# siyuanwu99/pred-occ-planner

Hardware: AMD Instinct MI355X
Metric: replans/sec (SOGM update + QP: full replan = SOGM update + A* + corridors + QP + deconfliction), 128-agent batch per GPU, 200x200x200x20 voxel grid; aggregate over all agents (higher is better)
Workload: dtype f32 occupancy / f64 planning; 1 GPU; 128 agents/GPU x 1 GPU, 200x200x200x20 SOGM, sim_fkpcp-style moving cylinders, batched ADMM QP (BASELINE configs[2] per GPU); agents_total=128, cloud_points=622040, cylinders=555, map_input_staleness_ticks=0, parallelism=agents sharded x1, 1 all-gather/tick, exchange=local, sogm_grids_per_agent=3, sogm_reset=sparse (logged 32-byte sectors), sogm_cell_order=2x2x2 tiles, map_update=at the start of the tick

## Files before the change

### pred-occ-planner_amd/csrc/sogm_device.hpp

```cpp
#pragma once

#include <hip/hip_fp16.h>
#include <hip/hip_runtime.h>

#include <cstdlib>

#include <new>
#include <stdint.h>

#include "../../include/sogm_abi_debug.h"
#include "../../include/sogm_detmath.h"
#include "sogm_gridpool.hpp"
#include "sogm_resources.hpp"

namespace sogm {
typedef float vfloat4 __attribute__((ext_vector_type(4)));

struct GridGeom {
  int   L, W, H, T;
  int   V;
  float res;
  float rx, ry, rz;
  float dt;
  float risk_threshold;
// ... 391 lines not shown
  for (int k = 0; k < piece; ++k) t0 += r.duration[k];
  const double tf = t0 + r.duration[piece], dur = tf - t0, s = (tt - t0) / dur;
  const double A[5][5] = {{1, -4, 6, -4, 1}, {0, 4, -12, 12, -4}, {0, 0, 6, -12, 6},
                          {0, 0, 0, 4, -4},  {0, 0, 0, 0, 1}};
  const double S0[5] = {1, s, s * s, s * s * s, (s * s) * (s * s)};
  const double S1[5] = {0, 1, 2 * s, 3 * (s * s), 4 * (s * s * s)};
  const double S2[5] = {0, 0, 2, 6 * s, 12 * (s * s)};
  const double *c    = r.cpts + piece * 15;
  for (int d = 0; d < 3; ++d) {
    double p = 0, v = 0, a = 0;
    for (int j = 0; j < 5; ++j) {
      double b = 0;
      for (int q = 0; q < 5; ++q) b += c[q * 3 + d] * A[q][j];
      p += b * S0[j];
      v += b * S1[j];
      a += b * S2[j];
    }
    out[d]     = p;
    out[3 + d] = v / dur;
    out[6 + d] = a / (dur * dur);
  }
  return true;
}
__device__ inline bool traj_eval_record(const SogmTrajRecord &r, double t_abs, double out[9]) {
  return traj_eval_relative(r, t_abs - r.time_start, out);
}
}

#define SOGM_TUNING_TABLE(X)                                                                                             \
  X(GROUPS, "groups", 2, 1, 64)                     \
  X(SPEC_ASTAR, "spec_astar", 1, 0, 1)             \
  X(CLEAR_GATE_FRAC, "clear_gate_frac", 1, 0, 1)  \
  X(QP_WGS, "qp_wgs", 0, 0, 1024)                     \
  X(FINISH_WGS, "finish_wgs", 0, 0, 64)             \
  X(CORRIDOR_WGS, "corridor_wgs", 0, 0, 65536)      \
  X(QP_ABLATE, "qp_ablate", 0, 0, 255)               \
  X(CLEAR_WGS, "clear_wgs", 0, 0, 65536)               \
  X(CLEAR_THROTTLE, "clear_throttle", 0, 0, 64)     \
  X(CLEAR_NT, "clear_nt", 1, 0, 1)                 \
  X(CLEAR_WIDE_WGS, "clear_wide_wgs", 256, 0, 65536)   \
  X(CLEAR_WIDE_BOUND, "clear_wide_bound", 0, 0, 64)  \
  X(CLEAR_HEAD_GB, "clear_head_gb", 1.0e9, 0, 1.0e12)   \
  X(CLEAR_EARLY, "clear_early", 0, 0, 1)           \
  X(CLEAR_RETIRE_AT_END, "clear_retire_at_end", 0, 0, 1)   \
  X(RESET_WGS, "reset_wgs", 32, 0, 4096)              \
  X(RESET_LANES, "reset_lanes", 0, 0, 4)           \
  X(RESET_UNROLL, "reset_unroll", 0, 0, 8)         \
  X(RESET_LATE, "reset_late", 1, 0, 1)             \
  X(STAMP_WGS, "stamp_wgs", 256, 0, 4096)             \
  X(STAMP_BITS_WGS, "stamp_bits_wgs", 0, 0, 4096)     \
  X(STAMP_LDS_LOG, "stamp_lds_log", 1, 0, 1)          \
  X(STAMP_CACHED, "stamp_cached", 0, 0, 1)            \
  X(STAMP_LDS_KB, "stamp_lds_kb", 0, 0, 64)                \
  X(SPLAT_WGS, "splat_wgs", 256, 0, 65536)             \
  X(SPLAT_OVERLAP, "splat_overlap", 1, 0, 1)       \
  X(PRESTAMP_BITS, "prestamp_bits", 32, 0, 1024)      \
  X(PRESTAMP_MARKS, "prestamp_marks", 64, 0, 1024)    \
  X(PRESTAMP_WGS, "prestamp_wgs", 0, 0, 65536)         \
  X(PRESTAMP_GATE_FRAC, "prestamp_gate_frac", 0.9, 0, 1)  \
  X(PRESTAMP_STREAM, "prestamp_stream", 1, 0, 1)  \
  X(PRESTAMP_LATE_AGENTS, "prestamp_late_agents", 8, 0, 65536)    \
  X(PRESTAMP_LATE_BITS, "prestamp_late_bits", 128, 0, 4096)      \
  X(PRESTAMP_LATE_MARKS, "prestamp_late_marks", 256, 0, 4096)    \
  X(FLIGHT_QP_UNITS, "flight_qp_units", 4, 1, 13)            \
  X(FLIGHT_SEARCH_UNITS, "flight_search_units", 2, 1, 13)    \
  X(FLIGHT_MAP_UNITS, "flight_map_units", 4, 1, 13)          \
  X(FLIGHT_MASKS, "flight_masks", 1, 0, 1)                   \
  X(FLIGHT_SPEC, "flight_spec", 1, 0, 1)                     \
  X(FLIGHT_RESET, "flight_reset", 8, 1, 256)                 \
  X(FLIGHT_BITS, "flight_bits", 16, 1, 256)                  \
  X(FLIGHT_MARKS, "flight_marks", 32, 1, 256)                \
  X(FLIGHT_SPLAT, "flight_splat", 4, 1, 64)                  \
  X(FLIGHT_ADMIT, "flight_admit", 48, 1, 65536)              \
  X(FLIGHT_PACE_US, "flight_pace_us", 20, 0, 100000)         \
  X(FLIGHT_HEADS, "flight_heads", 32, 1, 4096)               \
  X(FLIGHT_URGENT, "flight_urgent", 8, 0, 65536)            \
  X(FLIGHT_URGENT_WAVES, "flight_urgent_waves", 4096, 1, 4096)  \
  X(FLIGHT_URGENT_FINE, "flight_urgent_fine", 4, 1, 16)      \
  X(FLIGHT_GATE_PACE_US, "flight_gate_pace_us", 20, 0, 100000)   \
  X(FLIGHT_NEIGHBOUR_LAG, "flight_neighbour_lag", 2, 1, 2)  \
  X(FLIGHT_ENGINES, "flight_engines", 4, 1, 4)              \
  X(FLIGHT_ENGINE_FIRST, "flight_engine_first", 0, 0, 3)    \
  X(FLIGHT_EXCHANGE_UNITS, "flight_exchange_units", 0, 0, 4)  \
  X(FLIGHT_LIGHT_PER_CU, "flight_light_per_cu", 4, 1, 4)    \
  X(FLIGHT_MAP_PER_CU, "flight_map_per_cu", 8, 1, 8)        \
  X(UPDATE_FLOW, "update_flow", 0, 0, 1)                    \
  X(UPDATE_BITS, "update_bits", 16, 1, 256)                  \
  X(UPDATE_MARKS, "update_marks", 64, 1, 256)                \
  X(UPDATE_SPLAT, "update_splat", 40, 1, 64)                 \
  X(UPDATE_WGS, "update_wgs", 0, 0, 65536)                   \
  X(UPDATE_CHUNK, "update_chunk", 1, 1, 64)                  \
  X(UPDATE_CACHED, "update_cached", 0, 0, 1)                 \
  X(UPDATE_ORDER, "update_order", 1, 0, 1)
enum {
#define X(id, name, dflt, lo, hi) SOGM_TUNE_##id,
  SOGM_TUNING_TABLE(X)
#undef X
  SOGM_TUNE_N
};

struct sogm_ctx {
  sogm::Resources res;
  SogmSpec       spec;
  sogm::GridGeom geom;
  int            n_agents;
  int            device;
// ... 177 lines not shown
```

### pred-occ-planner_amd/csrc/sogm_map.hip

```cpp
#include <hip/hip_runtime.h>

#include <utility>
#include <vector>

#include "sogm_device.hpp"
#include "sogm_fsm.hpp"
#include "sogm_planner.hpp"

namespace sogm {

#define SOGM_MAX_CYL_LDS 1024

__device__ inline void cross3f(const float a[3], const float b[3], float o[3]) {
  o[0] = a[1] * b[2] - a[2] * b[1];
  o[1] = a[2] * b[0] - a[0] * b[2];
  o[2] = a[0] * b[1] - a[1] * b[0];
}
__device__ inline void quat_rotate_f(float qw, const float qv[3], const float v[3], float o[3]) {
  float uv[3], w2[3];
  cross3f(qv, v, uv);
  for (int k = 0; k < 3; ++k) uv[k] += uv[k];
  cross3f(qv, uv, w2);
  for (int k = 0; k < 3; ++k) o[k] = (v[k] + qw * uv[k]) + w2[k];
}
// ... 244 lines not shown
  if (f.cb.bounds) {
    stamp_bits_blocks<WAVE_DEDUPE>(g, f.cloud, f.cb, agent, sub, n_sub, pose[0], pose[1], pose[2], mask, lane);
  } else {
    const int begin = f.cloud_range[agent * 2], end = f.cloud_range[agent * 2 + 1];
    stamp_bits_range(g, f.cloud, begin + sub * 64 + lane, end, n_sub * 64, pose[0], pose[1], pose[2], mask);
  }
}
__global__ __launch_bounds__(64) void k_stamp_bits(GridGeom g, const float *__restrict__ cloud,
                                                   const int32_t *__restrict__ cloud_range,
                                                   const float *__restrict__ poses, unsigned *__restrict__ bits,
                                                   int words_per_agent, int agent0) {
  const MapFrame  f{.cloud = cloud, .cloud_range = cloud_range, .cb = {}};
  const MapTarget t{.bits = bits, .words = words_per_agent, .poses = const_cast<float *>(poses)};
  bits_ticket(g, f, t, (int)blockIdx.y + agent0, (int)blockIdx.x, (int)gridDim.x, (int)threadIdx.x);
}

__global__ __launch_bounds__(64) void k_stamp_bits_blocks(GridGeom g, const float *__restrict__ cloud, CloudBlocks cb,
                                                          const float *__restrict__ poses, unsigned *__restrict__ bits,
                                                          int words_per_agent) {
  const MapFrame  f{.cloud = cloud, .cb = cb};
  const MapTarget t{.bits = bits, .words = words_per_agent, .poses = const_cast<float *>(poses)};
  bits_ticket<true>(g, f, t, (int)blockIdx.y, (int)blockIdx.x, (int)gridDim.x, (int)threadIdx.x);
}
__global__ __launch_bounds__(64) void k_block_bounds(const float *__restrict__ cloud, int n_points, int block_points,
                                                     float *__restrict__ out) {
  const int b = blockIdx.x, lane = threadIdx.x;
  const int beg = b * block_points, end = beg + block_points < n_points ? beg + block_points : n_points;
  float xlo = INFINITY, xhi = -INFINITY, ylo = INFINITY, yhi = -INFINITY;
  for (int j = beg + lane; j < end; j += 64) {
    const float x = cloud[(size_t)j * 3], y = cloud[(size_t)j * 3 + 1];
    xlo = fminf(xlo, x);
    xhi = fmaxf(xhi, x);
    ylo = fminf(ylo, y);
    yhi = fmaxf(yhi, y);
  }
#pragma unroll
  for (int d = 32; d >= 1; d >>= 1) {
    xlo = fminf(xlo, __shfl_xor(xlo, d, 64));
    xhi = fmaxf(xhi, __shfl_xor(xhi, d, 64));
    ylo = fminf(ylo, __shfl_xor(ylo, d, 64));
    yhi = fmaxf(yhi, __shfl_xor(yhi, d, 64));
  }
  if (lane == 0) reinterpret_cast<float4 *>(out)[b] = make_float4(xlo, xhi, ylo, yhi);
}

#ifdef SOGM_PROFILE_PRESTAMP
__device__ unsigned long long g_ps_prof[12];
#define PS_CLK() wall_clock64()
#define PS_ADD(i, v) do { if (threadIdx.x == 0) atomicAdd(&g_ps_prof[i], (unsigned long long)(v)); } while (0)
#else
#define PS_CLK() 0ll
#define PS_ADD(i, v) do { } while (0)
#endif
template <bool CACHED>
__device__ __forceinline__ void stamp_marks_trips(const GridGeom &g, void *__restrict__ grid,
                                                  unsigned *__restrict__ bits, int words_per_agent,
                                                  const SogmCylinder *__restrict__ cyl, int n_cyl,
                                                  const float *__restrict__ poses,
                                                  const CylCand *__restrict__ cand_all,
                                                  const int *__restrict__ n_cand, int agent, const MarkLog &lg,
                                                  int w_first, int w_stride, CylCand *cand_lds = nullptr,
                                                  int cand_lds_cap = 0, unsigned *lds_secs = nullptr) {
  const int      kept   = n_cand[agent];
  const bool     culled = kept <= SOGM_MAX_CYL_LDS;
  const int      n_lds  = culled ? kept : 0;
  const int      n_loop = culled ? kept : n_cyl;
  const CylCand *cand   = cand_all + (size_t)agent * SOGM_MAX_CYL_LDS;
  const float   *pose   = poses + agent * 3;
  const float    p0 = pose[0], p1 = pose[1], p2 = pose[2];
  char          *base = reinterpret_cast<char *>(grid) + (size_t)agent * g.T * (size_t)g.V * (g.half ? 2 : 4);
  unsigned      *mask = bits + (size_t)agent * words_per_agent;
  const int      lane = threadIdx.x;
  unsigned n_marks = 0, n_logged = 0;
  int n_staged = 0;
  bool staged  = cand_lds == nullptr;
  for (int w0 = w_first; w0 < words_per_agent; w0 += w_stride) {
    uint4 *wp = reinterpret_cast<uint4 *>(mask + w0) + lane;
    uint4  w4 = *wp;
    if ((w4.x | w4.y | w4.z | w4.w) != 0u) *wp = make_uint4(0u, 0u, 0u, 0u);
    const int c0 = __popc(w4.x), c1 = c0 + __popc(w4.y), c2 = c1 + __popc(w4.z), cnt = c2 + __popc(w4.w);
    int       inc = cnt;
#pragma unroll
    for (int d = 1; d < 64; d <<= 1) {
      const int o = __shfl_up(inc, d, 64);
      if (lane >= d) inc += o;
    }
    const int excl  = inc - cnt;
    const int total = __shfl(inc, 63, 64);
    if (total > 0 && !staged) {
      n_staged            = n_lds < cand_lds_cap ? n_lds : cand_lds_cap;
      const uint4 *src    = reinterpret_cast<const uint4 *>(cand);
      uint4       *dst    = reinterpret_cast<uint4 *>(cand_lds);
      const int    pieces = n_staged * (int)(sizeof(CylCand) / 16);
      for (int q = lane; q < pieces; q += 64) dst[q] = src[q];
      __syncthreads();
      staged = true;
    }
    for (int b0 = 0; b0 < total; b0 += 64) {
      const int  i      = b0 + lane;
      const bool active = i < total;
      int lo = 0, hi = 63;
#pragma unroll
      for (int it = 0; it < 6; ++it) {
        const int mid = (lo + hi + 1) >> 1;
        const int em  = __shfl(excl, mid, 64);
        if (em <= i) lo = mid; else hi = mid - 1;
      }
      const int      own = lo;
      const int      r   = i - __shfl(excl, own, 64);
      const unsigned q0 = (unsigned)__shfl((int)w4.x, own, 64), q1 = (unsigned)__shfl((int)w4.y, own, 64);
      const unsigned q2 = (unsigned)__shfl((int)w4.z, own, 64), q3 = (unsigned)__shfl((int)w4.w, own, 64);
      const int      k0 = __shfl(c0, own, 64), k1 = __shfl(c1, own, 64), k2 = __shfl(c2, own, 64);
      const int esh = g.half ? 4 : 3;
      int       v   = 0;
      if (active) {
        const int sel = r < k0 ? 0 : r < k1 ? 1 : r < k2 ? 2 : 3;
        unsigned  wv  = sel == 0 ? q0 : sel == 1 ? q1 : sel == 2 ? q2 : q3;
        int       rr  = r - (sel == 0 ? 0 : sel == 1 ? k0 : sel == 2 ? k1 : k2);
        while (rr-- > 0) wv &= wv - 1;
        v = (w0 + own * 4 + sel) * 32 + __builtin_ctz(wv);
      }
      if (active) {
        cell_st(base, (size_t)v, 1.0F, g.half);
        ++n_marks;
      }
      float cx, cy, cz;
      g.corner_of(g.logical_of(v), pose, cx, cy, cz);
      float vx = 0.f, vy = 0.f;
      bool found = !active;
      [[maybe_unused]] const long long ps_w0 = PS_CLK();
      auto walk_filtered = [&](const auto *cl) __attribute__((always_inline)) {
        float xlo = active ? cx : INFINITY, xhi = active ? cx : -INFINITY;
        float ylo = active ? cy : INFINITY, yhi = active ? cy : -INFINITY;
#pragma unroll
        for (int d = 32; d >= 1; d >>= 1) {
          xlo = fminf(xlo, __shfl_xor(xlo, d, 64));
          xhi = fmaxf(xhi, __shfl_xor(xhi, d, 64));
          ylo = fminf(ylo, __shfl_xor(ylo, d, 64));
          yhi = fmaxf(yhi, __shfl_xor(yhi, d, 64));
        }
        bool done = false;
        for (int c0 = 0; c0 < n_loop && !done; c0 += 64) {
          bool maybe = false;
          if (c0 + lane < n_loop) {
            const CylCand cc = cl[c0 + lane];
            if (cc.type == 3) {
              const float ex = fmaxf(fmaxf(xlo - cc.x, cc.x - xhi), 0.0F), ey = fmaxf(fmaxf(ylo - cc.y, cc.y - yhi), 0.0F);
              maybe          = (double)sqrtf(ex * ex + ey * ey) <= cc.wlim + 0.01;
            } else {
              maybe = cc.type == 2;
            }
          }
          unsigned long long m = __ballot(maybe);
          while (m) {
            const int c = c0 + __builtin_ctzll(m);
            m &= m - 1;
            const CylCand cc = cl[c];
            if (!found) {
              bool hit = false;
              if (cc.type == 2) {
                hit = ring_contains(cyl[cc.orig], cx, cy, cz, g.res);
              } else if (cc.type == 3) {
                const float dx = cx - cc.x, dy = cy - cc.y, dz = cz - cz;
                const float dist = sqrtf(dx * dx + dy * dy + dz * dz);
                hit = (double)dist <= cc.wlim;
              }
              if (hit) {
                vx    = cc.vx;
                vy    = cc.vy;
                found = true;
              }
            }
            if (__builtin_amdgcn_readfirstlane((int)(__ballot(!found) == 0ull))) {
              done = true;
              break;
            }
          }
        }
      };
      if (cand_lds != nullptr && n_staged == n_loop) {
        walk_filtered(cand_lds);
      } else if (culled) {
        walk_filtered(cand);
      } else {
        for (int c0 = 0; c0 < n_loop; c0 += 4) {
          if (__builtin_amdgcn_readfirstlane((int)(__ballot(!found) == 0ull))) break;
          int    type[4], orig[4];
          float  ox[4], oy[4], wx[4], wy[4];
          double wlim[4];
  #pragma unroll
          for (int u = 0; u < 4; ++u) {
            const int c = c0 + u < n_loop ? c0 + u : n_loop - 1;
            if (c < n_lds) {
              const CylCand cc = c < n_staged ? cand_lds[c] : cand[c];
              type[u] = cc.type;
              orig[u] = cc.orig;
              ox[u]   = cc.x;
              oy[u]   = cc.y;
              wx[u]   = cc.vx;
              wy[u]   = cc.vy;
              wlim[u] = cc.wlim;
            } else {
              type[u] = cyl[c].type;
              orig[u] = c;
              ox[u]   = (float)cyl[c].x;
              oy[u]   = (float)cyl[c].y;
              wx[u]   = (float)cyl[c].vx;
              wy[u]   = (float)cyl[c].vy;
              wlim[u] = cyl[c].w + (double)g.clearance;
            }
          }
  #pragma unroll
          for (int u = 0; u < 4; ++u) {
            if (found || c0 + u >= n_loop) continue;
            bool hit = false;
            if (type[u] == 2) {
              hit = ring_contains(cyl[orig[u]], cx, cy, cz, g.res);
            } else if (type[u] == 3) {
              const float dx = cx - ox[u], dy = cy - oy[u], dz = cz - cz;
              const float dist = sqrtf(dx * dx + dy * dy + dz * dz);
              hit = (double)dist <= wlim[u];
            }
            if (hit) {
              vx    = wx[u];
              vy    = wy[u];
              found = true;
            }
          }
        }
      }
// ... 28 lines not shown
      constexpr int SG = 8;
      unsigned     *lent = lg.entries ? lg.entries + (size_t)agent * lg.cap : nullptr;
      unsigned p_secs[SG], p_keep = 0, p_off = 0;
      int      p_n = 0;
      auto     flush = [&]() __attribute__((always_inline)) {
        unsigned off = (unsigned)__shfl((int)p_off, 0, 64);
#pragma unroll
        for (int q = 0; q < SG; ++q)
          if (q < p_n) {
            const bool               mine = ((p_keep >> q) & 1u) != 0;
            const unsigned long long m    = __ballot(mine);
            const unsigned           li   = off + (unsigned)__popcll(m & lt);
            if (mine && li < (unsigned)lg.cap) lent[li] = p_secs[q];
            off += (unsigned)__popcll(m);
          }
      };
      for (int k0 = 0; k0 < g.T; k0 += SG) {
        unsigned secs[SG];
        unsigned keepbits = 0, run = 0;
#pragma unroll
        for (int q = 0; q < SG; ++q) {
          const int k = k0 + q;
          secs[q]     = 0xFFFFFFFFu;
          if (k < g.T) {
            const int    fv = k == 0 ? v : future_cell(k);
            const bool   in = k == 0 ? true : fv < g.V;
            const size_t ci = (size_t)k * g.V + (in ? fv : 0);
            if (k != 0 && active && in) {
              cell_st(base, ci, 1.0F, g.half);
              ++n_marks;
            }
            if (lent) {
              secs[q]                    = in ? (unsigned)(ci >> esh) : 0xFFFFFFFFu;
              const unsigned long long m = keep_of(secs[q], in);
              keepbits |= (unsigned)((m >> lane) & 1ull) << q;
              run += (unsigned)__popcll(m);
            }
          }
        }
        if (lent) {
          unsigned off = 0;
          if (lane == 0 && run) off = atomicAdd(lg.n + agent, run);
          n_logged += run;
          if (p_n) flush();
#pragma unroll
          for (int q = 0; q < SG; ++q) p_secs[q] = secs[q];
          p_keep = keepbits;
          p_off  = off;
          p_n    = g.T - k0 < SG ? g.T - k0 : SG;
        }
      }
      if (lent && p_n) flush();
      } else {
        unsigned *lent = lg.entries ? lg.entries + (size_t)agent * lg.cap : nullptr;
        unsigned  pref = 0, run = 0;
        constexpr unsigned NOT_KEPT = 0xFFFFFFFEu;
        {
          const unsigned long long m = keep_of((unsigned)v >> esh, true);
          run                        = (unsigned)__popcll(m);
          if (lds_secs) lds_secs[lane] = ((m >> lane) & 1ull) ? (unsigned)v >> esh : NOT_KEPT;
        }
        for (int k = 1; k < g.T; ++k) {
          const int    fv = future_cell(k);
          const bool   in = fv < g.V;
          const size_t ci = (size_t)k * g.V + (in ? fv : 0);
          if (active && in) {
            cell_st(base, ci, 1.0F, g.half);
            ++n_marks;
          }
          if (lent) {
            const unsigned long long m = keep_of(in ? (unsigned)(ci >> esh) : 0xFFFFFFFFu, in);
            if (lane == (k & 63)) pref = run;
            run += (unsigned)__popcll(m);
            if (lds_secs) lds_secs[k * 64 + lane] = ((m >> lane) & 1ull) ? (unsigned)(ci >> esh) : NOT_KEPT;
          }
        }
        if (lent && g.T <= 64) {
          unsigned lbase = 0;
          if (lane == 0) lbase = atomicAdd(lg.n + agent, run);
          lbase          = (unsigned)__shfl((int)lbase, 0, 64);
          n_logged += run;
          if (lds_secs) {
            for (int k = 0; k < g.T; ++k) {
              const unsigned           sec  = lds_secs[k * 64 + lane];
              const bool               mine = sec != NOT_KEPT;
              const unsigned long long m    = __ballot(mine);
              const unsigned           li   = lbase + (unsigned)__shfl((int)pref, k, 64) + (unsigned)__popcll(m & lt);
              if (mine && li < (unsigned)lg.cap) lent[li] = sec;
            }
          } else
          for (int k = 0; k < g.T; ++k) {
            const int                fv  = k == 0 ? v : future_cell(k);
            const bool               in  = fv < g.V;
            const unsigned           sec = in ? (unsigned)(((size_t)k * g.V + fv) >> esh) : 0xFFFFFFFFu;
            const unsigned long long m   = keep_of(sec, in);
            const unsigned           li  = lbase + (unsigned)__shfl((int)pref, k, 64) + (unsigned)__popcll(m & lt);
            if (((m >> lane) & 1ull) && li < (unsigned)lg.cap) lent[li] = sec;
          }
        } else if (lent && lane == 0) {
          atomicMax(lg.n + agent, (unsigned)lg.cap + 1u);
        }
      }
      PS_ADD(6, PS_CLK() - ps_w1);
    }
  }
  if (lg.stat) {
    for (int d = 32; d >= 1; d >>= 1) n_marks += (unsigned)__shfl_xor((int)n_marks, d, 64);
    if (lane == 0 && n_marks) {
      atomicAdd(lg.stat, (unsigned long long)n_marks);
      atomicAdd(lg.stat + 1, (unsigned long long)n_logged);
    }
  }
}
template <bool CACHED>
__device__ __forceinline__ void marks_ticket(const GridGeom &g, const MapFrame &f, const MapTarget &t, int agent, int sub,
                                             int n_sub, CylCand *cand_lds = nullptr, int cand_lds_cap = 0,
                                             unsigned *lds_secs = nullptr) {
  stamp_marks_trips<CACHED>(g, t.grid, t.bits, t.words, f.cyl, f.n_cyl, t.poses, (const CylCand *)t.cand, t.n_cand, agent, t.lg,
                            sub * 256, n_sub * 256, cand_lds, cand_lds_cap, lds_secs);
  if (cand_lds) __syncthreads();
}

__global__ __launch_bounds__(64) void k_stamp_marks(GridGeom g, void *__restrict__ grid,
                                                    unsigned *__restrict__ bits, int words_per_agent,
                                                    const SogmCylinder *__restrict__ cyl, int n_cyl,
                                                    const float *__restrict__ poses,
                                                    const CylCand *__restrict__ cand_all,
                                                    const int *__restrict__ n_cand, int agent0, MarkLog lg, int lds_log) {
  extern __shared__ unsigned s_marks_secs[];
  const MapFrame  f{.cyl = cyl, .n_cyl = n_cyl};
  const MapTarget t{.grid = grid, .bits = bits, .words = words_per_agent, .cand = const_cast<CylCand *>(cand_all),
                    .n_cand = const_cast<int *>(n_cand), .lg = lg, .poses = const_cast<float *>(poses)};
  marks_ticket<false>(g, f, t, (int)blockIdx.y + agent0, (int)blockIdx.x, (int)gridDim.x, nullptr, 0,
                      lds_log ? s_marks_secs : nullptr);
}
__global__ __launch_bounds__(64) void k_stamp_marks_cached(GridGeom g, void *__restrict__ grid,
                                                           unsigned *__restrict__ bits, int words_per_agent,
                                                           const SogmCylinder *__restrict__ cyl, int n_cyl,
                                                           const float *__restrict__ poses,
                                                           const CylCand *__restrict__ cand_all,
                                                           const int *__restrict__ n_cand, int agent0, MarkLog lg) {
  const MapFrame  f{.cyl = cyl, .n_cyl = n_cyl};
  const MapTarget t{.grid = grid, .bits = bits, .words = words_per_agent, .cand = const_cast<CylCand *>(cand_all),
                    .n_cand = const_cast<int *>(n_cand), .lg = lg, .poses = const_cast<float *>(poses)};
  marks_ticket<true>(g, f, t, (int)blockIdx.y + agent0, (int)blockIdx.x, (int)gridDim.x);
}

__device__ inline unsigned log_reserve(const MarkLog &lg, int agent, unsigned count) {
  const int                lane = (int)(threadIdx.x & 63);
  const unsigned long long lt   = lane ? (~0ull >> (64 - lane)) : 0ull;
  unsigned long long       todo = __ballot(1);
  unsigned                 base = 0;
  while (todo) {
    const int                leader = __ffsll((long long)todo) - 1;
    const int                la     = __shfl(agent, leader, 64);
    const unsigned long long grp    = __ballot(agent == la) & todo;
    unsigned                 b      = 0;
    if (lane == leader) b = atomicAdd(lg.n + la, count * (unsigned)__popcll(grp));
    b = (unsigned)__shfl((int)b, leader, 64);
    if (agent == la) base = b + count * (unsigned)__popcll(grp & lt);
    todo &= ~grp;
  }
  return base;
}

__device__ inline void splat_item(const GridGeom &g, void *__restrict__ grid, const SogmTrajRecord &R, int agent,
                                  int t, const int32_t *__restrict__ ego_ids, const float *__restrict__ poses,
                                  const double *__restrict__ stamps, const double *__restrict__ body, int n_body,
                                  const MarkLog &lg) {
  const int    esh   = g.half ? 4 : 3;
  const size_t tslab = (size_t)t * g.V;
  unsigned    *lent  = lg.entries ? lg.entries + (size_t)agent * lg.cap : nullptr;
  if (R.n_pieces <= 0 || R.drone_id == ego_ids[agent]) return;
  double time_end = R.time_start;
  for (int k = 0; k < R.n_pieces; ++k) time_end += R.duration[k];
  const double stamp = stamps[agent];
  const double t0    = stamp + (double)(g.dt * (float)0);
  const double tt    = stamp + (double)(g.dt * (float)t);
  if (g.map_kind == SOGM_MAP_RISKVOXEL) {
    for (int s_ = 0; s_ < t; ++s_) {
      const double ts = stamp + (double)(g.dt * (float)s_);
      if (!((R.time_start < ts && time_end > ts) || R.time_start > ts)) return;
    }
    const float *pose = poses + agent * 3;
    const double q0 = (double)pose[0], q1 = (double)pose[1], q2 = (double)pose[2];
    char        *slab = reinterpret_cast<char *>(grid) + ((size_t)agent * g.T + t) * (size_t)g.V * (g.half ? 2 : 4);
    double       p[3];
// ... 139 lines not shown
    const int  s   = tl % per;
    long long *pts = fc.ts + 8 * (size_t)ps.n_agents + 4 * (size_t)agent;
    if (s == 0) {
      [[maybe_unused]] const long long ps_c0 = PS_CLK();
      if (lane == 0) pts[0] = wall_clock64();
      stage_record_hover(&s_rec, s_hov, ps.tick.own, ps.tick.hover, agent, lane);
      if (lane == 0) {
        tick_inputs_agent(s_rec, s_hov, agent, ps.stamp, ps.tick, ps.tgt.poses);
        ps.tgt.stamps[agent] = ps.stamp;
        if (ps.poses_host)
          for (int k = 0; k < 3; ++k) ps.poses_host[agent * 3 + k] = ps.tgt.poses[agent * 3 + k];
      }
      __threadfence();
      __syncthreads();
      cull_ticket(g, ps.frame, ps.tgt, agent, ps.tgt.poses[agent * 3], ps.tgt.poses[agent * 3 + 1], lane);
      __threadfence();
      if (lane == 0) {
        pts[1] = wall_clock64();
        atomicAdd(&fc.stage[agent], 1);
      }
      PS_ADD(2, PS_CLK() - ps_c0);
    }
    [[maybe_unused]] const long long ps_t1 = PS_CLK();
    if (s < n_bits) {
      if (flow_wait_count(&fc.stage[agent], 1, &fc.hdr[FLOW_ERR])) break;
      [[maybe_unused]] const long long ps_t2 = PS_CLK();
      PS_ADD(1, ps_t2 - ps_t1);
      bits_ticket(g, ps.frame, ps.tgt, agent, s, n_bits, lane);
      __threadfence();
      PS_ADD(3, PS_CLK() - ps_t2);
      if (lane == 0 && atomicAdd(&fc.stage[agent], 1) + 1 == 1 + n_bits) pts[2] = wall_clock64();
    } else {
      if (flow_wait_count(&fc.stage[agent], 1 + n_bits, &fc.hdr[FLOW_ERR])) break;
      [[maybe_unused]] const long long ps_t2 = PS_CLK();
      PS_ADD(1, ps_t2 - ps_t1);
      marks_ticket<true>(g, ps.frame, ps.tgt, agent, s - n_bits, n_marks, s_cand, PRESTAMP_CAND_LDS);
      __threadfence();
      PS_ADD(4, PS_CLK() - ps_t2);
      if (lane == 0 && atomicAdd(&fc.stage[agent], 1) + 1 == 1 + n_bits + n_marks) {
        pts[3] = wall_clock64();
        __hip_atomic_store(&fc.stage[agent], FLOW_PS_DONE, __ATOMIC_RELEASE, __HIP_MEMORY_SCOPE_AGENT);
      }
    }
  }
}
#ifdef SOGM_PROFILE_PRESTAMP
}
extern "C" int sogm_debug_prestamp_prof(unsigned long long *out12_host, int reset) {
  if (hipDeviceSynchronize() != hipSuccess) return -1;
  if (out12_host && hipMemcpyFromSymbol(out12_host, HIP_SYMBOL(sogm::g_ps_prof), sizeof(unsigned long long) * 12) != hipSuccess) return -1;
  if (reset) {
    unsigned long long z[12] = {0};
    if (hipMemcpyToSymbol(HIP_SYMBOL(sogm::g_ps_prof), z, sizeof(z)) != hipSuccess) return -1;
  }
  return 0;
}
namespace sogm {
#endif
__device__ __forceinline__ MapFrame flight_frame(const FlightMapDev &d, int kl) {
  const FlightWorld &w = d.worlds[kl];
  MapFrame f{.cloud = w.cloud, .cloud_range = nullptr, .cb = d.cb, .cyl = w.cyl, .n_cyl = w.n_cyl};
  f.cb.bounds       = w.bounds;
  f.cb.n_blocks     = w.n_blocks;
  f.cb.block_points = w.block_points;
  f.cb.n_points     = w.n_points;
  return f;
}
__device__ __forceinline__ void flight_reset_ticket(char *__restrict__ base, size_t agent_bytes, const unsigned *__restrict__ e,
                                                    unsigned n, int cap, int first, int stride, int lane,
                                                    unsigned long long *__restrict__ stat) {
  const vfloat4 z = {0.f, 0.f, 0.f, 0.f};
  if (n > (unsigned)cap) {
    const size_t nv = agent_bytes / 16;
    for (size_t i = (size_t)first * 64 + lane; i < nv; i += (size_t)stride * 64)
      __builtin_nontemporal_store(z, reinterpret_cast<vfloat4 *>(base) + i);
    return;
  }
  const int part = lane & 1, pair = lane >> 1;
  unsigned  n_lines = 0;
  constexpr int U = 8;
  const size_t  step = (size_t)stride * 32;
  for (size_t i0 = (size_t)first * 32; i0 < n; i0 += U * step) {
    unsigned sct[U];
#pragma unroll
    for (int u = 0; u < U; ++u) {
      const size_t i = i0 + u * step + pair;
      sct[u]         = i < n ? e[i] : 0xFFFFFFFFu;
    }
#pragma unroll
    for (int u = 0; u < U; ++u) {
      const unsigned prev = __shfl_up(sct[u], 2);
      if (sct[u] == 0xFFFFFFFFu || (pair > 0 && prev == sct[u])) continue;
      const size_t off = (size_t)sct[u] * 32 + 16 * part;
      if (off + 16 <= agent_bytes) *reinterpret_cast<vfloat4 *>(base + off) = z;
      if (part == 0) ++n_lines;
    }
  }
  if (stat) {
    for (int d = 32; d >= 1; d >>= 1) n_lines += (unsigned)__shfl_xor((int)n_lines, d, 64);
    if (lane == 0 && n_lines) atomicAdd(stat + 2, (unsigned long long)n_lines * 32ull);
  }
}
__global__ __launch_bounds__(64) void k_flight_map(GridGeom g, FlightCtl fl, FlightMapDev d, unsigned long long *reset_stat) {
  __shared__ __attribute__((aligned(16))) SogmTrajRecord s_rec;
  __shared__ double                                      s_hov[9];
  __shared__ __attribute__((aligned(16))) CylCand        s_cand[PRESTAMP_CAND_LDS];
// ... 296 lines not shown
  hipLaunchKernelGGL(k_cull_cylinders, dim3(c->n_agents), dim3(64), 0, st, c->geom, f.cyl, f.n_cyl, poses, (CylCand *)tgt.cand,
                     tgt.n_cand, stamps, tgt.poses, tgt.stamps, f.cb, c->h_tick_clock);
}
static int launch_update_flow(sogm_ctx *c, hipStream_t st, const MapFrame &f, const MapTarget &tgt, const OverlayIO *ov) {
  if (int rc = update_flow_setup(c)) return rc;
  const int           A = c->n_agents;
  const UpdateFlowDev u{.tgt       = tgt,
                        .frame     = f,
                        .ov        = ov ? *ov : OverlayIO{},
                        .n_agents  = A,
                        .n_bits    = c->tune_i(SOGM_TUNE_UPDATE_BITS),
                        .n_marks   = c->tune_i(SOGM_TUNE_UPDATE_MARKS),
                        .n_splat   = ov && ov->n_rec > 0 ? c->tune_i(SOGM_TUNE_UPDATE_SPLAT) : 0,
                        .ctl       = c->d_update_ctl,
                        .chunk     = c->tune_i(SOGM_TUNE_UPDATE_CHUNK) > 0 ? c->tune_i(SOGM_TUNE_UPDATE_CHUNK) : 1,
                        .ts        = c->d_update_ts,
                        .map_ready = c->d_map_ready,
                        .epoch     = ++c->map_epoch,
                        .order     = c->d_update_order};
  int n_cu = 256;
  (void)hipDeviceGetAttribute(&n_cu, hipDeviceAttributeMultiprocessorCount, c->device);
  int       wgs   = c->tune_i(SOGM_TUNE_UPDATE_WGS) > 0 ? c->tune_i(SOGM_TUNE_UPDATE_WGS) : 16 * n_cu;
  const int total = A * (u.n_bits + u.n_marks + u.n_splat);
  if (wgs > total) wgs = total;
  SOGM_HIP_CHECK(hipEventRecord(c->ev_uin, st));
  SOGM_HIP_CHECK(hipStreamWaitEvent(c->ustream, c->ev_uin, 0));
  SOGM_HIP_CHECK(hipMemsetAsync(c->d_update_ctl, 0, sizeof(int) * UpdateBlock::words(A), c->ustream));
  if (c->tune_i(SOGM_TUNE_UPDATE_CACHED))
    hipLaunchKernelGGL(k_update_flow<true>, dim3(wgs), dim3(64), 0, c->ustream, c->geom, u);
  else
    hipLaunchKernelGGL(k_update_flow<false>, dim3(wgs), dim3(64), 0, c->ustream, c->geom, u);
  SOGM_HIP_CHECK(hipGetLastError());
  prof_end(c, SOGM_PROF_STAMP, c->ustream);
  SOGM_HIP_CHECK(hipEventRecord(c->ev_udone, c->ustream));
  c->update_pending = 1;
  return SOGM_OK;
}
static void launch_stamp(sogm_ctx *c, hipStream_t st, const MapFrame &f, const MapTarget &tgt) {
  const int A         = c->n_agents;
  const int stamp_wgs = c->tune_i(SOGM_TUNE_STAMP_WGS) > 0 ? c->tune_i(SOGM_TUNE_STAMP_WGS) : 256;
  const int bits_wgs  = c->tune_i(SOGM_TUNE_STAMP_BITS_WGS) > 0 ? c->tune_i(SOGM_TUNE_STAMP_BITS_WGS) : stamp_wgs;
  if (f.cb.bounds)
    hipLaunchKernelGGL(k_stamp_bits_blocks, dim3(bits_wgs, A), dim3(64), 0, st, c->geom, f.cloud, f.cb, tgt.poses, tgt.bits,
                       tgt.words);
  else
    hipLaunchKernelGGL(k_stamp_bits, dim3(bits_wgs, A), dim3(64), 0, st, c->geom, f.cloud, f.cloud_range, tgt.poses, tgt.bits,
                       tgt.words, 0);
  const size_t marks_lds = (size_t)c->tune_i(SOGM_TUNE_STAMP_LDS_KB) * 1024;
  if (c->tune_i(SOGM_TUNE_STAMP_CACHED)) {
    hipLaunchKernelGGL(k_stamp_marks_cached, dim3(stamp_wgs, A), dim3(64), marks_lds, st, c->geom, tgt.grid, tgt.bits,
                       tgt.words, f.cyl, f.n_cyl, tgt.poses, (const CylCand *)tgt.cand, (const int *)tgt.n_cand, 0, tgt.lg);
  } else {
    const int    lds_log = tgt.lg.entries && c->spec.T <= 64 && c->tune_i(SOGM_TUNE_STAMP_LDS_LOG) ? 1 : 0;
    const size_t lds     = marks_lds + (lds_log ? sizeof(unsigned) * 64 * (size_t)c->spec.T : 0);
    hipLaunchKernelGGL(k_stamp_marks, dim3(stamp_wgs, A), dim3(64), lds, st, c->geom, tgt.grid, tgt.bits, tgt.words, f.cyl,
                       f.n_cyl, tgt.poses, (const CylCand *)tgt.cand, (const int *)tgt.n_cand, 0, tgt.lg, lds_log);
  }
}
static int launch_overlay(sogm_ctx *c, hipStream_t st, const OverlayIO &ov, const int *wait_stage, int *wait_err,
                          int max_workgroups) {
  const long long total = (long long)c->n_agents * ov.n_rec * c->spec.T;
  long long       nblk  = (total + 255) / 256;
  if (max_workgroups > 0 && nblk > max_workgroups) nblk = max_workgroups;
  prof_begin(c, SOGM_PROF_SPLAT, st);
  hipLaunchKernelGGL(k_splat_neighbours, dim3((unsigned)nblk), dim3(256), 0, st, c->geom, (void *)c->d_grid, ov.rec, ov.n_rec,
                     ov.ego_ids, c->d_poses, c->d_stamps, ov.body, ov.n_body, c->n_agents, 0, mark_log(c, c->pool.current()),
                     wait_stage, wait_err);
  prof_end(c, SOGM_PROF_SPLAT, st);
  SOGM_HIP_CHECK(hipGetLastError());
  return SOGM_OK;
}
static OverlayIO overlay_io(const sogm_ctx *c, const SogmTrajRecord *records, int n_records, const int32_t *ego_ids) {
  return OverlayIO{.rec = records, .n_rec = n_records, .ego_ids = ego_ids, .body = c->d_body, .n_body = c->n_body};
}

static int update_maps(sogm_ctx *c, hipStream_t st, MapFrame frame, const SogmWorld *world, const float *poses,
                       const double *stamps, const OverlayIO *ov) {
  SOGM_HIP_CHECK(hipSetDevice(c->device));
  if (int rc = update_joins(c, st, world, ov != nullptr, &frame.cb)) return rc;
  if (int rc = take_grid(c, st)) return rc;
  MapTarget tgt{};
  if (int rc = map_target(c, c->pool.current(), false, st, &tgt)) return rc;
  c->n_stamps++;
  prof_begin(c, SOGM_PROF_STAMP, st);
  launch_cull(c, st, frame, tgt, poses, stamps);
  if (world && c->tune_i(SOGM_TUNE_UPDATE_FLOW) != 0) {
    if (int rc = launch_update_flow(c, st, frame, tgt, ov)) return rc;
  } else {
    launch_stamp(c, st, frame, tgt);
    prof_end(c, SOGM_PROF_STAMP, st);
    SOGM_HIP_CHECK(hipGetLastError());
    if (ov && ov->n_rec > 0)
      if (int rc = launch_overlay(c, st, *ov, nullptr, nullptr, 0)) return rc;
  }
  c->updated = 1;
  return SOGM_OK;
}

}

using namespace sogm;

extern "C" {

int sogm_update_gt(sogm_ctx *c, const float *cloud_xyz, const int32_t *cloud_range,
                   const SogmCylinder *cylinders, int n_cyl, const float *poses,
                   const double *stamps, void *stream) {
  if (!c || !cloud_xyz || !cloud_range || !poses || !stamps || n_cyl < 0 ||
      (n_cyl > 0 && !cylinders))
// ... 123 lines not shown
```

Before: 13500 replans/s.

## Restructure stamp-marks kernel with multi-wave workgroups, prefetch and register-broadcast candidates

Rewrites k_stamp_marks so each workgroup can hold several 64-lane waves, each taking its own stride of mask words. Candidates can optionally be staged into LDS once per workgroup. Inside the trip loop, the next mask word and the next batch of cylinder candidates are prefetched into registers, and the candidate fields are broadcast with readlane instead of reloading from memory. Optional profiling counters are added under a compile flag. With the defaults (1 wave, cand LDS 0) the launch shape is unchanged, but the prefetch and readlane paths now always run, adding register pressure and an extra load per trip.

```diff
diff --git a/pred-occ-planner_amd/csrc/sogm_device.hpp b/pred-occ-planner_amd/csrc/sogm_device.hpp
--- a/pred-occ-planner_amd/csrc/sogm_device.hpp
+++ b/pred-occ-planner_amd/csrc/sogm_device.hpp
@@ -467,6 +467,8 @@
   X(STAMP_LDS_LOG, "stamp_lds_log", 1, 0, 1)          \
   X(STAMP_CACHED, "stamp_cached", 0, 0, 1)            \
   X(STAMP_LDS_KB, "stamp_lds_kb", 0, 0, 64)                \
+  X(STAMP_WG_WAVES, "stamp_wg_waves", 1, 1, 12)            \
+  X(STAMP_CAND_LDS, "stamp_cand_lds", 0, 0, 1024)          \
   X(SPLAT_WGS, "splat_wgs", 256, 0, 65536)             \
   X(SPLAT_OVERLAP, "splat_overlap", 1, 0, 1)       \
   X(PRESTAMP_BITS, "prestamp_bits", 32, 0, 1024)      \
diff --git a/pred-occ-planner_amd/csrc/sogm_map.hip b/pred-occ-planner_amd/csrc/sogm_map.hip
--- a/pred-occ-planner_amd/csrc/sogm_map.hip
+++ b/pred-occ-planner_amd/csrc/sogm_map.hip
@@ -320,7 +320,19 @@
 #define PS_CLK() 0ll
 #define PS_ADD(i, v) do { } while (0)
 #endif
-template <bool CACHED>
+#ifdef SOGM_PROFILE_STAMP
+__device__ unsigned long long g_sm_prof[16];
+#define SM_CLK() wall_clock64()
+#define SM_DECL(...) __VA_ARGS__
+#define SM_USE(x) asm volatile("" ::"v"(x))
+#define SM_USE_S(x) asm volatile("" ::"s"(x))
+#else
+#define SM_CLK() 0ll
+#define SM_DECL(...)
+#define SM_USE(x) do { } while (0)
+#define SM_USE_S(x) do { } while (0)
+#endif
+template <bool CACHED, bool LOCKSTEP = false>
 __device__ __forceinline__ void stamp_marks_trips(const GridGeom &g, void *__restrict__ grid,
                                                   unsigned *__restrict__ bits, int words_per_agent,
                                                   const SogmCylinder *__restrict__ cyl, int n_cyl,
@@ -328,7 +340,7 @@
                                                   const CylCand *__restrict__ cand_all,
                                                   const int *__restrict__ n_cand, int agent, const MarkLog &lg,
                                                   int w_first, int w_stride, CylCand *cand_lds = nullptr,
-                                                  int cand_lds_cap = 0, unsigned *lds_secs = nullptr) {
+                                                  int cand_lds_cap = 0, unsigned *lds_secs = nullptr, int n_prestaged = 0) {
   const int      kept   = n_cand[agent];
   const bool     culled = kept <= SOGM_MAX_CYL_LDS;
   const int      n_lds  = culled ? kept : 0;
@@ -338,13 +350,24 @@
   const float    p0 = pose[0], p1 = pose[1], p2 = pose[2];
   char          *base = reinterpret_cast<char *>(grid) + (size_t)agent * g.T * (size_t)g.V * (g.half ? 2 : 4);
   unsigned      *mask = bits + (size_t)agent * words_per_agent;
-  const int      lane = threadIdx.x;
+  const int      lane = LOCKSTEP ? (int)(threadIdx.x & 63u) : (int)threadIdx.x;
   unsigned n_marks = 0, n_logged = 0;
-  int n_staged = 0;
-  bool staged  = cand_lds == nullptr;
+  int n_staged = LOCKSTEP ? n_prestaged : 0;
+  bool staged  = LOCKSTEP || cand_lds == nullptr;
+  uint4 w4_next = make_uint4(0u, 0u, 0u, 0u);
+  if constexpr (LOCKSTEP)
+    if (w_first < words_per_agent) w4_next = reinterpret_cast<const uint4 *>(mask + w_first)[lane];
+  SM_DECL(long long sm[14] = {0, 0, 0, 0, 0, 0, 0, 0, 0, 0, 0, 0, 0, 0}; const long long sm_in = SM_CLK();)
   for (int w0 = w_first; w0 < words_per_agent; w0 += w_stride) {
+    SM_DECL(const long long sm_t = SM_CLK();)
     uint4 *wp = reinterpret_cast<uint4 *>(mask + w0) + lane;
-    uint4  w4 = *wp;
+    uint4  w4;
+    if constexpr (LOCKSTEP) {
+      w4 = w4_next;
+      if (w0 + w_stride < words_per_agent) w4_next = reinterpret_cast<const uint4 *>(mask + w0 + w_stride)[lane];
+    } else {
+      w4 = *wp;
+    }
     if ((w4.x | w4.y | w4.z | w4.w) != 0u) *wp = make_uint4(0u, 0u, 0u, 0u);
     const int c0 = __popc(w4.x), c1 = c0 + __popc(w4.y), c2 = c1 + __popc(w4.z), cnt = c2 + __popc(w4.w);
     int       inc = cnt;
@@ -355,6 +378,8 @@
     }
     const int excl  = inc - cnt;
     const int total = __shfl(inc, 63, 64);
+    SM_USE(total);
+    SM_DECL(sm[0] += SM_CLK() - sm_t; sm[10] += 1;)
     if (total > 0 && !staged) {
       n_staged            = n_lds < cand_lds_cap ? n_lds : cand_lds_cap;
       const uint4 *src    = reinterpret_cast<const uint4 *>(cand);
@@ -365,6 +390,7 @@
       staged = true;
     }
     for (int b0 = 0; b0 < total; b0 += 64) {
+      SM_DECL(const long long sm_c = SM_CLK();)
       const int  i      = b0 + lane;
       const bool active = i < total;
       int lo = 0, hi = 63;
@@ -397,7 +423,12 @@
       float vx = 0.f, vy = 0.f;
       bool found = !active;
       [[maybe_unused]] const long long ps_w0 = PS_CLK();
+      SM_USE(cx);
+      SM_USE(cy);
+      SM_DECL(const long long sm_w = SM_CLK(); sm[1] += sm_w - sm_c; sm[8] += 1;)
       auto walk_filtered = [&](const auto *cl) __attribute__((always_inline)) {
+        CylCand nb{};
+        if (lane < n_loop) nb = cl[lane];
         float xlo = active ? cx : INFINITY, xhi = active ? cx : -INFINITY;
         float ylo = active ? cy : INFINITY, yhi = active ? cy : -INFINITY;
 #pragma unroll
@@ -407,23 +438,40 @@
           ylo = fminf(ylo, __shfl_xor(ylo, d, 64));
           yhi = fmaxf(yhi, __shfl_xor(yhi, d, 64));
         }
+        SM_USE(xlo);
+        SM_USE(xhi);
+        SM_USE(ylo);
+        SM_USE(yhi);
+        SM_DECL(long long sm_b = SM_CLK(); sm[2] += sm_b - sm_w;)
         bool done = false;
         for (int c0 = 0; c0 < n_loop && !done; c0 += 64) {
+          const CylCand mine = nb;
+          if (c0 + 64 + lane < n_loop) nb = cl[c0 + 64 + lane];
           bool maybe = false;
           if (c0 + lane < n_loop) {
-            const CylCand cc = cl[c0 + lane];
-            if (cc.type == 3) {
-              const float ex = fmaxf(fmaxf(xlo - cc.x, cc.x - xhi), 0.0F), ey = fmaxf(fmaxf(ylo - cc.y, cc.y - yhi), 0.0F);
-              maybe          = (double)sqrtf(ex * ex + ey * ey) <= cc.wlim + 0.01;
+            if (mine.type == 3) {
+              const float ex = fmaxf(fmaxf(xlo - mine.x, mine.x - xhi), 0.0F), ey = fmaxf(fmaxf(ylo - mine.y, mine.y - yhi), 0.0F);
+              maybe          = (double)sqrtf(ex * ex + ey * ey) <= mine.wlim + 0.01;
             } else {
-              maybe = cc.type == 2;
+              maybe = mine.type == 2;
             }
           }
           unsigned long long m = __ballot(maybe);
+          SM_USE_S(m);
+          SM_DECL(const long long sm_s = SM_CLK(); sm[3] += sm_s - sm_b;)
+          const int wl_hi = __double2hiint(mine.wlim), wl_lo = __double2loint(mine.wlim);
           while (m) {
-            const int c = c0 + __builtin_ctzll(m);
+            const int src = __builtin_ctzll(m);
             m &= m - 1;
-            const CylCand cc = cl[c];
+            SM_DECL(sm[9] += 1;)
+            CylCand cc;
+            cc.type = __builtin_amdgcn_readlane(mine.type, src);
+            cc.orig = __builtin_amdgcn_readlane(mine.orig, src);
+            cc.x    = __int_as_float(__builtin_amdgcn_readlane(__float_as_int(mine.x), src));
+            cc.y    = __int_as_float(__builtin_amdgcn_readlane(__float_as_int(mine.y), src));
+            cc.vx   = __int_as_float(__builtin_amdgcn_readlane(__float_as_int(mine.vx), src));
+            cc.vy   = __int_as_float(__builtin_amdgcn_readlane(__float_as_int(mine.vy), src));
+            cc.wlim = __hiloint2double(__builtin_amdgcn_readlane(wl_hi, src), __builtin_amdgcn_readlane(wl_lo, src));
             if (!found) {
               bool hit = false;
               if (cc.type == 2) {
@@ -444,6 +492,7 @@
               break;
             }
           }
+          SM_DECL(sm_b = SM_CLK(); sm[4] += sm_b - sm_s;)
         }
       };
       if (cand_lds != nullptr && n_staged == n_loop) {
@@ -578,6 +627,7 @@
       }
       if (lent && p_n) flush();
       } else {
+        SM_DECL(const long long sm_st = SM_CLK(); sm[13] += sm_st - sm_w;)
         unsigned *lent = lg.entries ? lg.entries + (size_t)agent * lg.cap : nullptr;
         unsigned  pref = 0, run = 0;
         constexpr unsigned NOT_KEPT = 0xFFFFFFFEu;
@@ -601,10 +651,16 @@
             if (lds_secs) lds_secs[k * 64 + lane] = ((m >> lane) & 1ull) ? (unsigned)(ci >> esh) : NOT_KEPT;
           }
         }
+        SM_DECL(const long long sm_r = SM_CLK(); sm[5] += sm_r - sm_st;)
         if (lent && g.T <= 64) {
           unsigned lbase = 0;
           if (lane == 0) lbase = atomicAdd(lg.n + agent, run);
-          lbase          = (unsigned)__shfl((int)lbase, 0, 64);
+          if constexpr (LOCKSTEP)
+            lbase = (unsigned)__builtin_amdgcn_readfirstlane((int)lbase);
+          else
+            lbase = (unsigned)__shfl((int)lbase, 0, 64);
+          SM_USE(lbase);
+          SM_DECL(const long long sm_l = SM_CLK(); sm[6] += sm_l - sm_r;)
           n_logged += run;
           if (lds_secs) {
             for (int k = 0; k < g.T; ++k) {
@@ -623,6 +679,7 @@
             const unsigned           li  = lbase + (unsigned)__shfl((int)pref, k, 64) + (unsigned)__popcll(m & lt);
             if (((m >> lane) & 1ull) && li < (unsigned)lg.cap) lent[li] = sec;
           }
+          SM_DECL(sm[7] += SM_CLK() - sm_l;)
         } else if (lent && lane == 0) {
           atomicMax(lg.n + agent, (unsigned)lg.cap + 1u);
         }
@@ -630,6 +687,14 @@
       PS_ADD(6, PS_CLK() - ps_w1);
     }
   }
+#ifdef SOGM_PROFILE_STAMP
+  if constexpr (!CACHED) {
+    sm[11] = 1;
+    sm[12] = SM_CLK() - sm_in;
+    if (lane == 0)
+      for (int q = 0; q < 14; ++q) atomicAdd(&g_sm_prof[q], (unsigned long long)sm[q]);
+  }
+#endif
   if (lg.stat) {
     for (int d = 32; d >= 1; d >>= 1) n_marks += (unsigned)__shfl_xor((int)n_marks, d, 64);
     if (lane == 0 && n_marks) {
@@ -647,18 +712,33 @@
   if (cand_lds) __syncthreads();
 }
 
-__global__ __launch_bounds__(64) void k_stamp_marks(GridGeom g, void *__restrict__ grid,
+constexpr int STAMP_WG_WAVES_MAX = 12;
+__global__ __launch_bounds__(64 * STAMP_WG_WAVES_MAX) void k_stamp_marks(GridGeom g, void *__restrict__ grid,
                                                     unsigned *__restrict__ bits, int words_per_agent,
                                                     const SogmCylinder *__restrict__ cyl, int n_cyl,
                                                     const float *__restrict__ poses,
                                                     const CylCand *__restrict__ cand_all,
-                                                    const int *__restrict__ n_cand, int agent0, MarkLog lg, int lds_log) {
-  extern __shared__ unsigned s_marks_secs[];
-  const MapFrame  f{.cyl = cyl, .n_cyl = n_cyl};
-  const MapTarget t{.grid = grid, .bits = bits, .words = words_per_agent, .cand = const_cast<CylCand *>(cand_all),
-                    .n_cand = const_cast<int *>(n_cand), .lg = lg, .poses = const_cast<float *>(poses)};
-  marks_ticket<false>(g, f, t, (int)blockIdx.y + agent0, (int)blockIdx.x, (int)gridDim.x, nullptr, 0,
-                      lds_log ? s_marks_secs : nullptr);
+                                                    const int *__restrict__ n_cand, int agent0, MarkLog lg, int lds_log,
+                                                    int n_sub, int cand_cap) {
+  extern __shared__ uint4 s_marks_lds[];
+  CylCand   *s_cand = reinterpret_cast<CylCand *>(s_marks_lds);
+  unsigned  *s_secs = reinterpret_cast<unsigned *>(s_marks_lds + (size_t)cand_cap * (sizeof(CylCand) / 16));
+  const int  agent  = (int)blockIdx.y + agent0;
+  const int  wave = (int)(threadIdx.x >> 6), waves = (int)(blockDim.x >> 6);
+  int        n_staged = 0;
+  if (cand_cap > 0) {
+    const int kept = n_cand[agent];
+    if (kept <= SOGM_MAX_CYL_LDS) n_staged = kept < cand_cap ? kept : cand_cap;
+    const uint4 *src    = reinterpret_cast<const uint4 *>(cand_all + (size_t)agent * SOGM_MAX_CYL_LDS);
+    const int    pieces = n_staged * (int)(sizeof(CylCand) / 16);
+    for (int q = (int)threadIdx.x; q < pieces; q += (int)blockDim.x) s_marks_lds[q] = src[q];
+    __syncthreads();
+  }
+  const int sub = (int)blockIdx.x * waves + wave;
+  if (sub >= n_sub) return;
+  stamp_marks_trips<false, true>(g, grid, bits, words_per_agent, cyl, n_cyl, poses, cand_all, n_cand, agent, lg, sub * 256,
+                                 n_sub * 256, cand_cap > 0 ? s_cand : nullptr, cand_cap,
+                                 lds_log ? s_secs + (size_t)wave * 64 * g.T : nullptr, n_staged);
 }
 __global__ __launch_bounds__(64) void k_stamp_marks_cached(GridGeom g, void *__restrict__ grid,
                                                            unsigned *__restrict__ bits, int words_per_agent,
@@ -904,6 +984,19 @@
   if (reset) {
     unsigned long long z[12] = {0};
     if (hipMemcpyToSymbol(HIP_SYMBOL(sogm::g_ps_prof), z, sizeof(z)) != hipSuccess) return -1;
+  }
+  return 0;
+}
+namespace sogm {
+#endif
+#ifdef SOGM_PROFILE_STAMP
+}
+extern "C" int sogm_debug_stamp_prof(unsigned long long *out16_host, int reset) {
+  if (hipDeviceSynchronize() != hipSuccess) return -1;
+  if (out16_host && hipMemcpyFromSymbol(out16_host, HIP_SYMBOL(sogm::g_sm_prof), sizeof(unsigned long long) * 16) != hipSuccess) return -1;
+  if (reset) {
+    unsigned long long z[16] = {0};
+    if (hipMemcpyToSymbol(HIP_SYMBOL(sogm::g_sm_prof), z, sizeof(z)) != hipSuccess) return -1;
   }
   return 0;
 }
@@ -1306,9 +1399,19 @@
                        tgt.words, f.cyl, f.n_cyl, tgt.poses, (const CylCand *)tgt.cand, (const int *)tgt.n_cand, 0, tgt.lg);
   } else {
     const int    lds_log = tgt.lg.entries && c->spec.T <= 64 && c->tune_i(SOGM_TUNE_STAMP_LDS_LOG) ? 1 : 0;
-    const size_t lds     = marks_lds + (lds_log ? sizeof(unsigned) * 64 * (size_t)c->spec.T : 0);
-    hipLaunchKernelGGL(k_stamp_marks, dim3(stamp_wgs, A), dim3(64), lds, st, c->geom, tgt.grid, tgt.bits, tgt.words, f.cyl,
-                       f.n_cyl, tgt.poses, (const CylCand *)tgt.cand, (const int *)tgt.n_cand, 0, tgt.lg, lds_log);
+    const size_t secs  = lds_log ? sizeof(unsigned) * 64 * (size_t)c->spec.T : 0;
+    int          waves = c->tune_i(SOGM_TUNE_STAMP_WG_WAVES) > 0 ? c->tune_i(SOGM_TUNE_STAMP_WG_WAVES) : 1;
+    if (waves > STAMP_WG_WAVES_MAX) waves = STAMP_WG_WAVES_MAX;
+    if (waves > stamp_wgs) waves = stamp_wgs;
+    int cand_cap = c->tune_i(SOGM_TUNE_STAMP_CAND_LDS);
+    if (cand_cap > SOGM_MAX_CYL_LDS) cand_cap = SOGM_MAX_CYL_LDS;
+    const size_t lds_max = 64 * 1024;
+    while (waves > 1 && sizeof(CylCand) * cand_cap + secs * waves + marks_lds > lds_max) --waves;
+    if (sizeof(CylCand) * cand_cap + secs * waves + marks_lds > lds_max) cand_cap = 0;
+    const size_t lds = sizeof(CylCand) * cand_cap + secs * waves + marks_lds;
+    hipLaunchKernelGGL(k_stamp_marks, dim3((stamp_wgs + waves - 1) / waves, A), dim3(64 * waves), lds, st, c->geom, tgt.grid,
+                       tgt.bits, tgt.words, f.cyl, f.n_cyl, tgt.poses, (const CylCand *)tgt.cand, (const int *)tgt.n_cand, 0,
+                       tgt.lg, lds_log, stamp_wgs, cand_cap);
   }
 }
 static int launch_overlay(sogm_ctx *c, hipStream_t st, const OverlayIO &ov, const int *wait_stage, int *wait_err,
```

After: 13470 replans/s. About the same (-0.2%).
